# brech1/keaki

Measured on AMD Instinct MI355X. Metric: BN254 G1 scalar-mults/sec on 2^24-point MSM (per GPU), higher is better.
Workload: dtype u32 limbs, 256-bit Montgomery modular integer (9 x 29-bit lazy limbs in the bucket kernel, 8 x 32 elsewhere)

## Files before the change

### bench_tools/dbg/sort_harness.hip

```cpp
#include <hip/hip_runtime.h>
#include <cstdio>
#include <vector>
#ifdef KEAKI_STAMP
__device__ unsigned long long g_stamp[4096];
#define STAMP(cond, i) do { if (cond) g_stamp[(i)] = __builtin_readcyclecounter(); } while (0)
#endif
#include "msm.hip.h"
using namespace bn254;
__global__ void k_fill(u32* p, size_t nwords) {
  size_t i = (size_t)blockIdx.x * blockDim.x + threadIdx.x;
  if (i >= nwords) return;
  unsigned long long z = (i + 1) * 0x9E3779B97F4A7C15ull;
  z = (z ^ (z >> 30)) * 0xBF58476D1CE4E5B9ull; z = (z ^ (z >> 27)) * 0x94D049BB133111EBull; z ^= z >> 31;
  u32 v = (u32)z;
  if ((i & 7) == 7) v &= 0x0FFFFFFFu;
  p[i] = v;
}
#define CK(x) do { hipError_t e_ = (x); if (e_ != hipSuccess) { printf("%s: %s\n", #x, hipGetErrorString(e_)); return 1; } } while (0)
int main(int argc, char** argv) {
  const int log2n = argc > 1 ? atoi(argv[1]) : 24;
  const size_t n = (size_t)1 << log2n;
  MsmPlan plan = msm_make_plan(n, 22);
  MsmShape s = plan.s; s.stride = (u32)n;
  size_t nb = plan.max_b;
  PartShape ps;
  if (!part_make_shape(n, s.W, nb, &ps, argc > 2 ? atoi(argv[2]) : -1, argc > 3 ? atoi(argv[3]) : -1, argc > 4 ? atoi(argv[4]) : -1)) { printf("shape\n"); return 1; }
  printf("n=2^%d W=%u c=%u nbins=%u shift=%u hb=%u nf=%u tile=%u ntiles=%u te=%u geom=%u\n", log2n, s.W, s.c, ps.nbins, ps.shift, ps.hb, ps.nf, ps.tile, ps.ntiles, ps.te, ps.geom);
  const size_t pairs = n * s.W;
  u32 *scal, *tiles, *sorted, *counts, *segoff, *bin_total; u16* tstart; uint2* cellmeta; BinMeta* bins; v4u_t* segtab;
  CK(hipMalloc(&scal, n * 32)); CK(hipMalloc(&tiles, (size_t)ps.ntiles * ps.te * 4)); CK(hipMalloc(&sorted, pairs * 4)); CK(hipMalloc(&counts, nb * 4));
  CK(hipMalloc(&segoff, part_max_chunks(pairs, ps.nbins) * ps.nf * 4)); CK(hipMalloc(&segtab, nb * 16)); CK(hipMalloc(&bin_total, ps.nbins * 4));
  CK(hipMalloc(&tstart, (size_t)ps.ntiles * (ps.nbins + 1) * 2)); CK(hipMalloc(&cellmeta, (size_t)ps.nbins * ps.ntiles * 8)); CK(hipMalloc(&bins, ps.nbins * sizeof(BinMeta)));
  hipLaunchKernelGGL(k_fill, dim3((n * 8 + 255) / 256), dim3(256), 0, 0, scal, n * 8);
  CK(hipDeviceSynchronize());
  hipEvent_t ev[6]; for (auto& e : ev) CK(hipEventCreate(&e));
  int ncu = 256;
  for (int it = 0; it < 4; it++) {
    CK(hipEventRecord(ev[0]));
    hipLaunchKernelGGL(k_tile_sort<12>, dim3(ps.ntiles < (u32)ncu ? ps.ntiles : ncu), dim3(T1_THREADS), 0, 0, (const Fr*)scal, s, ps, tiles, tstart);
    CK(hipEventRecord(ev[1]));
    hipLaunchKernelGGL(k_cell_prefix, dim3(ps.nbins), dim3(1024), 0, 0, (const u16*)tstart, ps, cellmeta, bin_total);
    CK(hipEventRecord(ev[2]));
    hipLaunchKernelGGL(k_bin_scan, dim3(1), dim3(1024), 0, 0, (const u32*)bin_total, ps.nbins, bins);
    CK(hipEventRecord(ev[3]));
#define CS(L, R, Q) hipLaunchKernelGGL((k_chunk_sort<L, R, Q>), dim3(ps.nbins), dim3(C2_THREADS), 0, 0, (const u32*)tiles, (const uint2*)cellmeta, (const BinMeta*)bins, s, ps, (u32)nb, sorted, segtab, segoff, counts)
    switch (ps.geom) { case 0: CS(8, 1, 16); break; case 1: CS(16, 1, 16); break; case 2: CS(16, 2, 8); break; default: CS(16, 4, 4); break; }
    CK(hipEventRecord(ev[4]));
    CK(hipDeviceSynchronize());
    float a, b, c, d;
    CK(hipEventElapsedTime(&a, ev[0], ev[1])); CK(hipEventElapsedTime(&b, ev[1], ev[2])); CK(hipEventElapsedTime(&c, ev[2], ev[3])); CK(hipEventElapsedTime(&d, ev[3], ev[4]));
    printf("tile_sort %.3f  cell_prefix %.3f  bin_scan %.3f  chunk_sort %.3f ms\n", a, b, c, d);
  }
  std::vector<u32> hc(nb); CK(hipMemcpy(hc.data(), counts, nb * 4, hipMemcpyDeviceToHost));
  unsigned long long tot = 0; for (u32 v : hc) tot += v;
  printf("sum of bucket counts %llu (pairs %zu minus zero digits)\n", tot, pairs);
#ifdef KEAKI_STAMP
  std::vector<unsigned long long> st(4096);
  CK(hipMemcpyFromSymbol(st.data(), HIP_SYMBOL(g_stamp), 4096 * 8));
  printf("chunk_sort stamps (one workgroup), cycles between marks per chunk:\n");
  for (int k = 0; k < 8; k++) {
    printf(" chunk %d:", k);
    for (int i = 1; i < 12; i++) { long long d = (long long)(st[k * 16 + i] - st[k * 16 + i - 1]); printf(" %lld", st[k * 16 + i] ? d : -1); }
    printf("  | slow=%llu odd lanes=%llu last odd grp/c0=%llx\n", st[k * 16 + 12], st[k * 16 + 13], st[k * 16 + 14]);
  }
  printf("tile_sort stamps (one workgroup, first tiles):\n");
  for (int k = 0; k < 4; k++) {
    printf(" tile %d:", k);
    for (int i = 1; i < 10; i++) { long long d = (long long)(st[2048 + k * 16 + i] - st[2048 + k * 16 + i - 1]); printf(" %lld", st[2048 + k * 16 + i] ? d : -1); }
// ... 6 lines not shown
```

### keaki_amd/csrc/api.hip

```cpp
#include "internal.h"

#include <algorithm>
#include <set>
#include <utility>
#include <vector>

using namespace keaki_internal;

struct keaki_hip_srs_g1 {
  const void* d = nullptr;
  size_t n = 0;
  bool owned = false;
  int device = -1;
  std::recursive_mutex mu;
  keaki_hip_ctx* acct = nullptr;
  size_t fk_bytes = 0;
  void* table = nullptr;
  size_t table_bytes = 0;
  int c_table = 0;
  void* fk_hat_s = nullptr;
  int fk_log2d = -1;
};
struct keaki_hip_srs_g2 {
  const void* d = nullptr;
// ... 312 lines not shown
#define KEAKI_SRC_HASH "unknown"
#endif
#ifdef KEAKI_DIAG
const char* keaki_hip_version(void) { return "keaki-hip 0.3 (gfx950) DIAGNOSTIC BUILD (diag_row_mask available: not the product) src=" KEAKI_SRC_HASH; }
#else
const char* keaki_hip_version(void) { return "keaki-hip 0.3 (gfx950) src=" KEAKI_SRC_HASH; }
#endif

extern "C++" {
namespace {
void tune_from_env(Tuning& t) {
  auto geti = [](const char* name, long long& out) { const char* e = getenv(name); if (!e || !*e) return false; out = atoll(e); return true; };
  long long v;
  if (geti("KEAKI_MSM_C", v)) t.msm_c = (int)v;
  if (geti("KEAKI_MSM_C_SHARED", v)) t.msm_c_shared = (int)v;
  if (geti("KEAKI_REDUCE_L", v)) t.reduce_l = (int)v;
  if (geti("KEAKI_PART_SHIFT", v)) t.part_shift = (int)v;
  if (geti("KEAKI_ACC_U29", v)) t.acc_u29 = v != 0;
  if (geti("KEAKI_ACC_U29_G2", v)) t.acc_u29_g2 = v != 0;
  if (geti("KEAKI_ACC_NT", v)) t.acc_nt = v != 0;
  if (geti("KEAKI_ACC_PREFETCH", v)) t.acc_prefetch = v != 0;
  if (geti("KEAKI_ACC_IDXQ", v)) t.acc_idxq = v != 0;
  if (geti("KEAKI_CS_MASKED", v)) t.cs_masked = v != 0;
  if (geti("KEAKI_FK_UNIFORM", v)) t.fk_uniform = v != 0;
  if (geti("KEAKI_FK_GTAB", v)) t.fk_gtab = v != 0;
  if (geti("KEAKI_FK_ADDSUB29", v)) t.fk_addsub29 = v != 0;
  if (geti("KEAKI_FK_RADIX4", v)) t.fk_radix4 = v != 0;
  if (geti("KEAKI_FB_OCC1", v)) t.fb_occ1 = v != 0;
  if (geti("KEAKI_MSM_SHORT_TABLES", v)) t.msm_short_tables = (int)v;
  if (geti("KEAKI_PAIR_WIDE_MAX", v)) t.pair_wide_max = (int)v;
  if (geti("KEAKI_PAIR_TWO_WAVES", v)) t.pair_two_waves = v != 0;
  if (geti("KEAKI_GT_WB_B", v)) t.gt_wb_b = (int)v;
  if (geti("KEAKI_ENCAP_GT", v)) t.encap_gt = v;
  if (geti("KEAKI_HOST_PREFAULT", v)) t.host_prefault = v != 0;
  if (geti("KEAKI_PIPE_CHUNKS", v)) t.pipe_chunks = v != 0;
  if (geti("KEAKI_MSM_PIPE_CHUNKS", v)) t.msm_pipe_chunks = (int)v;
  if (geti("KEAKI_MSM_PIPE_MIN", v)) t.msm_pipe_min = v;
  if (geti("KEAKI_MSM_PIPE_GROWTH", v)) t.msm_pipe_growth = (int)v;
}
struct BufClass { DevBuf* b; int cls; };
std::vector<BufClass> all_bufs(keaki_hip_ctx* ctx) {
  std::vector<BufClass> v;
  for (DevBuf* b : {&ctx->digits, &ctx->hist, &ctx->offsets, &ctx->cursor, &ctx->sorted, &ctx->buckets, &ctx->acc29, &ctx->partials, &ctx->wsums, &ctx->bsums,
                    &ctx->tmp_a, &ctx->tmp_b, &ctx->tmp_c, &ctx->io_a, &ctx->io_b, &ctx->io_c, &ctx->io_d, &ctx->io_e, &ctx->perm, &ctx->heavy,
                    &ctx->pair_ws, &ctx->verify_io, &ctx->g2gen_lines, &ctx->fk_tab, &ctx->g2pow_lines, &ctx->g2pow_pts})
    v.push_back({b, 1});
// ... 62 lines not shown
  thread_local std::string copy;
  keaki_hip_ctx* c = const_cast<keaki_hip_ctx*>(ctx);
  std::lock_guard<std::recursive_mutex> lock_(c->mu);
  copy = c->err;
  return copy.c_str();
}

keaki_status keaki_hip_ctx_set_option(keaki_hip_ctx* ctx, const char* name, int64_t value) {
  if (!ctx) return KEAKI_ERR_BAD_ARG;
  std::lock_guard<std::recursive_mutex> lock_(ctx->mu);
  if (!name) return fail(ctx, KEAKI_ERR_BAD_ARG, "ctx_set_option: name is null");
  Tuning& t = ctx->tune;
  const std::string k(name);
  if (k == "msm_c") t.msm_c = (int)value;
  else if (k == "msm_c_shared") t.msm_c_shared = (int)value;
  else if (k == "reduce_l") t.reduce_l = (int)value;
  else if (k == "part_shift") t.part_shift = (int)value;
  else if (k == "acc_u29") t.acc_u29 = value != 0;
  else if (k == "acc_u29_g2") t.acc_u29_g2 = value != 0;
  else if (k == "acc_nt") t.acc_nt = value != 0;
  else if (k == "acc_prefetch") t.acc_prefetch = value != 0;
  else if (k == "acc_idxq") t.acc_idxq = value != 0;
  else if (k == "cs_masked") t.cs_masked = value != 0;
  else if (k == "fk_uniform") t.fk_uniform = value != 0;
  else if (k == "fk_gtab") t.fk_gtab = value != 0;
  else if (k == "fk_addsub29") t.fk_addsub29 = value != 0;
  else if (k == "fk_radix4") t.fk_radix4 = value != 0;
  else if (k == "fb_occ1") t.fb_occ1 = value != 0;
  else if (k == "msm_short_tables") t.msm_short_tables = (int)value;
  else if (k == "pair_wide_max") t.pair_wide_max = (int)value;
  else if (k == "pair_two_waves") t.pair_two_waves = value != 0;
  else if (k == "gt_wb_b") {
    if (value != 0 && (value < 8 || value > 22 || gt_table_powers((uint32_t)value) > 320)) return fail(ctx, KEAKI_ERR_BAD_ARG, "ctx_set_option: gt_wb_b = %lld out of range", (long long)value);
    if ((int)value != t.gt_wb_b) { ctx->gt_b_ready = false; ctx->gt_b_fallback = false; }
    t.gt_wb_b = (int)value;
  } else if (k == "encap_gt") t.encap_gt = value;
  else if (k == "host_prefault") t.host_prefault = value != 0;
  else if (k == "pipe_chunks") t.pipe_chunks = value != 0;
#ifdef KEAKI_DIAG
  else if (k == "diag_row_mask") t.diag_row_mask = (unsigned)value;
#endif
  else if (k == "msm_pipe_chunks") t.msm_pipe_chunks = (int)value;
  else if (k == "msm_pipe_min") t.msm_pipe_min = value;
  else if (k == "msm_pipe_growth") t.msm_pipe_growth = (int)value;
  else return fail(ctx, KEAKI_ERR_BAD_ARG, "ctx_set_option: unknown option '%s'", name);
  return KEAKI_OK;
// ... 1084 lines not shown
```

### keaki_amd/csrc/internal.h

```cpp
#pragma once
#include <hip/hip_runtime.h>

#include <cstdarg>
#include <cstdio>
#include <cstdlib>
#include <atomic>
#include <cstring>
#include <functional>
#include <mutex>
#include <string>
#include <utility>
#include <vector>

#include "../../include/keaki_hip.h"

namespace keaki_internal {

struct DevBuf {
  void* p = nullptr;
  size_t cap = 0;
};

}

namespace keaki_internal {
struct Tuning {
  int msm_c = 0;
  int msm_c_shared = 0;
  int msm_short_tables = -1;
  int reduce_l = 0;
  int part_shift = -1;
  bool acc_u29 = true;
  bool acc_u29_g2 = true;
  bool acc_prefetch = true;
  bool acc_idxq = true;
  bool cs_masked = true;
  bool acc_nt = false;
  bool fk_uniform = true;
  bool fk_gtab = true;
  bool fk_radix4 = true;
  bool fk_addsub29 = true;
  bool fb_occ1 = false;
  int pair_wide_max = -1;
  bool pair_two_waves = true;
  int gt_wb_b = 0;
  long long encap_gt = -1;
  bool host_prefault = true;
  bool pipe_chunks = true;
  int msm_pipe_chunks = -1;
  long long msm_pipe_min = 1 << 20;
  int msm_pipe_growth = 160;
#ifdef KEAKI_DIAG
  unsigned diag_row_mask = 0;
#endif
  size_t alloc_limit = 0;
};
}

struct keaki_hip_ctx {
// ... 155 lines not shown
```

### keaki_amd/csrc/msm.hip.h

```cpp
#pragma once
#include <type_traits>
#include "bn254_curve.hip.h"
#include "fq29.hip.h"
#include "xyzz29.hip.h"
#include "jac29.hip.h"
#include "xyzz29_g2.hip.h"

namespace bn254 {

typedef uint16_t u16;
typedef u32 v4u_t __attribute__((ext_vector_type(4)));
constexpr u32 DIGIT_NONE = 0xFFFFFFFFu;
#ifndef STAMP
#define STAMP(cond, i) do { } while (0)
#endif

struct MsmShape {
  u32 n;
  u32 c;
  u32 W;
  u32 k;
  u32 stride;
};
KDEV u32 msm_width(const MsmShape& s, u32 w) { return w < s.k ? s.c : s.c - 1; }
// ... 63 lines not shown
#pragma unroll
  for (u32 w = 0; w < W; w++) {
    const u32 off = P::offset(w), wd = P::width(w), j = off >> 5, sh = off & 31;
    const u32 lo = v[j], hi = j + 1 < 8 ? v[j + 1] : 0u;
    const u32 d = (sh + wd <= 32 ? lo >> sh : __builtin_amdgcn_alignbit(hi, lo, sh)) & ((1u << wd) - 1u);
    const u32 full = 1u << wd, half = full >> 1;
    const u32 coef = d + carry;
    if (w == W - 1) {
      code[w] = coef ? coef - 1u : DIGIT_NONE;
    } else {
      const bool neg = coef > half;
      carry = neg ? 1u : 0u;
      code[w] = neg ? (coef != full ? ((full - coef - 1u) | 0x80000000u) : DIGIT_NONE) : (coef ? coef - 1u : DIGIT_NONE);
    }
  }
}

template <class Emit>
KDEV void msm_for_each_digit(const Fr& k, const MsmShape& s, Emit emit) {
  u32 v[8];
  fp_from_mont<FrParams>(v, k);
  msm_for_each_digit_canon(v, s, emit);
}

constexpr u32 T1_THREADS = 1024;
constexpr u32 T1_PER = 3;
constexpr u32 T1_CAP = 36864;
constexpr u32 PART_MAX_BINS = 2048;
constexpr u32 C2_THREADS = 1024;
constexpr u32 C2_CAP = 32768;
constexpr u32 PART_MAX_FINE_SHIFT = 11;
constexpr u32 PART_MAX_FINE = 1u << PART_MAX_FINE_SHIFT;
constexpr u32 SEG_INLINE = 4;
constexpr u32 TE_WPOS = 12, TE_SIGN = 19, TE_FINE = 20, TE_VALID = 0x80000000u;

struct PartShape {
  u32 nbins, lb;
  u32 shift, hb;
  u32 nf;
  u32 tile;
  u32 ntiles;
  u32 te;
  u32 geom;
};
KDEV u32 part_bin(const PartShape& ps, u32 g) { return (g >> ps.shift) & (ps.nbins - 1u); }
KDEV u32 part_fine(const PartShape& ps, u32 g) { return ((g >> (ps.shift + ps.lb)) << ps.shift) | (g & ((1u << ps.shift) - 1u)); }
// ... 127 lines not shown
          const u32 g = (s.stride ? 0u : msm_bucket_base(s, w)) + (cd & 0x7FFFFFFFu);
          const u32 pos = atomicAdd(&cur[ok ? part_bin(ps, g) : PART_MAX_BINS + (t & 63u)], 1u);
          ent[ok ? pos : T1_CAP + (t & 63u)] = TE_VALID | (part_fine(ps, g) << TE_FINE) | ((cd >> 31) << TE_SIGN) | (w << TE_WPOS) | li;
        }
      } else if (act[p]) {
        msm_for_each_digit_canon(canon[p], s, [&](u32 w, u32 cd) {
          const u32 g = (s.stride ? 0u : msm_bucket_base(s, w)) + (cd & 0x7FFFFFFFu);
          const u32 pos = atomicAdd(&cur[part_bin(ps, g)], 1u);
          ent[pos] = TE_VALID | (part_fine(ps, g) << TE_FINE) | ((cd >> 31) << TE_SIGN) | (w << TE_WPOS) | li;
        });
      }
    }
    STAMP(blockIdx.x == 100 && t == 0 && sk < 4, 2048 + sk * 16 + 5);
    lds_barrier();
    STAMP(blockIdx.x == 100 && t == 0 && sk < 4, 2048 + sk * 16 + 6);
    u32* dst = tiles + (size_t)tile * ps.te;
#pragma unroll 4
    for (u32 q = t; q < m; q += T1_THREADS) dst[q] = ent[q];
    STAMP(blockIdx.x == 100 && t == 0 && sk < 4, 2048 + sk * 16 + 7);
  }
}

static __global__ void __launch_bounds__(1024) k_cell_prefix(const u16* __restrict__ tstart, PartShape ps, uint2* __restrict__ cellmeta,
                                                             u32* __restrict__ bin_total) {
  __shared__ u32 a[4096];
  __shared__ u32 wsum[16];
  const u32 b = blockIdx.x, t = threadIdx.x;
  u32 carry = 0;
  for (u32 base = 0; base < ps.ntiles; base += 4096) {
    u32 st[4], ln[4];
#pragma unroll
    for (u32 k = 0; k < 4; k++) {
      const u32 tile = base + 4 * t + k;
      st[k] = 0; ln[k] = 0;
      if (tile < ps.ntiles) {
        const u16* row = tstart + (size_t)tile * (ps.nbins + 1) + b;
        st[k] = row[0];
        ln[k] = (u32)row[1] - st[k];
      }
      a[4 * t + k] = ln[k];
    }
    const u32 tot = lds_exclusive_scan4(a, 4096, wsum);
#pragma unroll
    for (u32 k = 0; k < 4; k++) {
      const u32 tile = base + 4 * t + k;
      if (tile < ps.ntiles) cellmeta[(size_t)b * ps.ntiles + tile] = make_uint2(carry + a[4 * t + k], st[k] | (ln[k] << 16));
    }
    carry += tot;
    lds_barrier();
  }
  if (t == 0) bin_total[b] = carry;
}
struct BinMeta {
  u32 img_base, chunk_first, nch, total;
};
static __global__ void __launch_bounds__(1024) k_bin_scan(const u32* __restrict__ bin_total, u32 nbins, BinMeta* __restrict__ bins) {
  __shared__ u32 a[2048];
  __shared__ u32 c[2048];
  __shared__ u32 wsum[16];
  const u32 t = threadIdx.x;
  u32 tt[2];
#pragma unroll
  for (u32 k = 0; k < 2; k++) {
    const u32 b = 2 * t + k;
    tt[k] = b < nbins ? bin_total[b] : 0u;
    a[b] = tt[k];
    c[b] = (tt[k] + C2_CAP - 1) / C2_CAP;
  }
  lds_exclusive_scan4(a, 2048, wsum);
  lds_exclusive_scan4(c, 2048, wsum);
#pragma unroll
  for (u32 k = 0; k < 2; k++) {
    const u32 b = 2 * t + k;
    if (b < nbins) bins[b] = {a[b], c[b], (tt[k] + C2_CAP - 1) / C2_CAP, tt[k]};
  }
}

constexpr u32 C2_META = 2048;
KDEV u32 chunk_payload(u32 en, u32 ibase, u32 stride) {
  return (((en >> TE_SIGN) & 1u) << 31) | (ibase + (en & ((1u << TE_WPOS) - 1u)) + ((en >> TE_WPOS) & ((1u << (TE_SIGN - TE_WPOS)) - 1u)) * stride);
}
template <int PHASE>
KDEV void chunk_slow(const u32* __restrict__ tiles, const uint2* __restrict__ cm, const PartShape& ps, u32 stride, u32 c0, u32 lo, u32 hi, u32* hist,
                     u32* pay, u32* sh_next) {
  const u32 grp = threadIdx.x >> 4, l16 = threadIdx.x & 15;
  for (u32 c = c0 + grp; c < ps.ntiles; c += C2_THREADS / 16) {
    const uint2 m = cm[c];
    const u32 len = m.y >> 16;
    if (PHASE == 0 && m.x + len > hi && l16 == 0) atomicMin(sh_next, c);
    if (m.x > hi || (m.x == hi && len)) break;
    const u32 j0 = m.x < lo ? lo - m.x : 0u, j1 = hi - m.x < len ? hi - m.x : len;
    const u32* src = tiles + (size_t)c * ps.te + (m.y & 0xFFFFu);
    for (u32 j = j0 + l16; j < j1; j += 16) {
      const u32 en = src[j];
      const u32 f = (en >> TE_FINE) & (PART_MAX_FINE - 1u);
      if (PHASE == 0) {
        atomicAdd(&hist[f], 1u);
      } else {
        const u32 pos = atomicAdd(&hist[f], 1u);
        pay[pos] = chunk_payload(en, c * ps.tile, stride);
      }
    }
  }
}
template <u32 L, u32 R, u32 Q, bool MASKED = true>
static __global__ void __launch_bounds__(C2_THREADS) k_chunk_sort(const u32* __restrict__ tiles, const uint2* __restrict__ cellmeta,
                                                                  const BinMeta* __restrict__ bins, MsmShape s, PartShape ps, u32 nbuckets_total,
                                                                  u32* __restrict__ sorted, v4u_t* __restrict__ segtab, u32* __restrict__ segoff,
                                                                  u32* __restrict__ bucket_counts) {
  constexpr u32 GROUPS = C2_THREADS / L, CELLS = GROUPS * Q, CAPC = 4 * L * R, NB = 4, QB = Q / NB;
  static_assert(CELLS <= C2_META && Q * R * 4 <= 64 && Q <= 32 && Q % NB == 0 && PART_MAX_FINE == 2 * C2_THREADS, "gather shape");
  __shared__ u32 pay[C2_CAP + 64];
  __shared__ uint2 meta[C2_META];
  __shared__ u32 hist[PART_MAX_FINE + 64];
  __shared__ u32 wsum[C2_THREADS / 64];
  __shared__ u32 sh_next, sh_odd;
  const u32 b = blockIdx.x, t = threadIdx.x, nf = ps.nf;
  const BinMeta bm = bins[b];
  const uint2* cm = cellmeta + (size_t)b * ps.ntiles;
  u32 tot[2] = {0, 0};
  u32 c0 = 0;
  for (u32 f = t; f < PART_MAX_FINE + 64; f += C2_THREADS) hist[f] = 0;
#pragma unroll
  for (u32 i = 0; i < C2_META / C2_THREADS; i++) {
    const u32 ci = t + i * C2_THREADS;
    if (ci < CELLS) meta[ci] = ci < ps.ntiles ? cm[ci] : make_uint2(0xFFFFFFFFu, 0u);
  }
  if (t == 0) { sh_next = ps.ntiles; sh_odd = 0; }
  lds_barrier();
  for (u32 k = 0; k < bm.nch; k++) {
    const u32 lo = k * C2_CAP, hi = bm.total - lo < C2_CAP ? bm.total : lo + C2_CAP;
    u32 tk = t;
    asm volatile("" : "+v"(tk));
    const u32 grp = tk / L, ll = tk % L, dummy = PART_MAX_FINE + (tk & 63u);
    STAMP(b == 100 && t == 0 && k < 8, k * 16 + 0);
    const size_t span = (size_t)(ps.ntiles - c0) * ps.te * 4;
    const __amdgpu_buffer_rsrc_t img = __builtin_amdgcn_make_buffer_rsrc((void*)(tiles + (size_t)c0 * ps.te), 0,
                                                                       span < 0xFFFFFFF0ull ? (u32)span : 0xFFFFFFF0u, 0x00020000);
    auto fetch = [&](u32 tt, u32 q0, u32 (&e)[QB][R][4], u32& longcells, u32& cand, bool& odd) {
      const u32 grp = tt / L, ll = tt % L;
#pragma unroll
// ... 149 lines not shown
    STAMP(b == 100 && t == 0 && k < 8, k * 16 + 7);
    u32 tw = threadIdx.x;
    asm volatile("" : "+v"(tw));
    u32* dst = sorted + bm.img_base + lo;
#pragma unroll 4
    for (u32 q = tw; q < hi - lo; q += C2_THREADS) dst[q] = pay[q];
    for (u32 f = tw; f < PART_MAX_FINE + 64; f += C2_THREADS) hist[f] = 0;
    if (k + 1 < bm.nch) {
#pragma unroll
      for (u32 i = 0; i < C2_META / C2_THREADS; i++) if (tw + i * C2_THREADS < CELLS) meta[tw + i * C2_THREADS] = mnext[i];
    }
    if (t == 0) { sh_next = ps.ntiles; sh_odd = 0; }
    c0 = c_next;
    STAMP(b == 100 && t == 0 && k < 8, k * 16 + 8);
    lds_barrier();
  }
  u32 te = threadIdx.x;
  asm volatile("" : "+v"(te));
#pragma unroll
  for (u32 i = 0; i < 2; i++) {
    const u32 f = 2 * te + i, g = part_bucket(ps, b, f);
    if (f < nf && g < nbuckets_total) {
      bucket_counts[g] = tot[i];
      for (u32 kk = bm.nch; kk < SEG_INLINE; kk++) reinterpret_cast<u32*>(segtab)[(size_t)g * SEG_INLINE + kk] = 0u;
    }
  }
}

struct SortView {
  const u32* sorted;
  const BinMeta* bins;
  const v4u_t* segtab;
  const u32* segoff;
  PartShape ps;
};
struct SegWalker {
  u32 pos, left;
  u32 w0, w1, w2, w3;
  u32 c, nch;
  u32 img_base, o;
};
KDEV void seg_init(SegWalker& w, const SortView& v, u32 t) {
  const BinMeta bm = v.bins[part_bin(v.ps, t)];
  const v4u_t sw = v.segtab[t];
  w.w0 = sw[0]; w.w1 = sw[1]; w.w2 = sw[2]; w.w3 = sw[3];
  w.img_base = bm.img_base;
  w.o = bm.chunk_first * v.ps.nf + part_fine(v.ps, t);
  w.nch = bm.nch;
// ... 74 lines not shown
  __shared__ u32 wsum[SCAN_THREADS / 64];
  u32 lane = threadIdx.x & 63, wid = threadIdx.x >> 6;
  u32 x = v;
#pragma unroll
  for (int o = 1; o < 64; o <<= 1) {
    u32 y = __shfl_up(x, o, 64);
    if (lane >= (u32)o) x += y;
  }
  if (lane == 63) wsum[wid] = x;
  __syncthreads();
  u32 base = 0, tot = 0;
#pragma unroll
  for (u32 k = 0; k < SCAN_THREADS / 64; k++) {
    u32 s = wsum[k];
    if (k < wid) base += s;
    tot += s;
  }
  __syncthreads();
  *total = tot;
  return base + x - v;
}


constexpr u32 CNT_BINS = 1024;
constexpr u32 HEAVY_MIN = 8192, HEAVY_SLICE = 16384;
struct HeavyList {
  u32 n;
  u32 nslices;
};
static __global__ void __launch_bounds__(256) k_cnt_hist(const u32* __restrict__ counts, u32 nb, u32* __restrict__ ghist, HeavyList* __restrict__ hv,
                                                         u32 hv_cap, u32 hv_slice_cap, u32* __restrict__ hv_bucket, u32* __restrict__ hv_first,
                                                         u32* __restrict__ hv_owner) {
  __shared__ u32 h[CNT_BINS];
  for (u32 b = threadIdx.x; b < CNT_BINS; b += 256) h[b] = 0;
  __syncthreads();
  const u32 base = blockIdx.x * 1024;
  for (u32 t = threadIdx.x; t < 1024; t += 256) {
    u32 g = base + t;
    if (g < nb) {
      u32 c = counts[g];
      atomicAdd(&h[c < CNT_BINS - 1 ? c : CNT_BINS - 1], 1u);
      if (c >= HEAVY_MIN) {
        const u32 nsl = (c + HEAVY_SLICE - 1) / HEAVY_SLICE;
        const u32 slot = atomicAdd(&hv->n, 1u);
        if (slot < hv_cap) {
          const u32 first = atomicAdd(&hv->nslices, nsl);
          hv_bucket[slot] = g;
          hv_first[slot] = first;
          for (u32 k = 0; k < nsl && first + k < hv_slice_cap; k++) hv_owner[first + k] = slot;
        }
      }
    }
  }
  __syncthreads();
  for (u32 b = threadIdx.x; b < CNT_BINS; b += 256) if (h[b]) atomicAdd(&ghist[b], h[b]);
}
static __global__ void __launch_bounds__(CNT_BINS) k_cnt_offsets(const u32* __restrict__ ghist, u32* __restrict__ start) {
  __shared__ u32 sh[CNT_BINS];
  u32 b = threadIdx.x;
  sh[b] = ghist[CNT_BINS - 1 - b];
  __syncthreads();
  for (u32 o = 1; o < CNT_BINS; o <<= 1) {
    u32 v = b >= o ? sh[b - o] : 0u;
    __syncthreads();
    sh[b] += v;
    __syncthreads();
  }
  start[CNT_BINS - 1 - b] = sh[b] - ghist[CNT_BINS - 1 - b];
}
static __global__ void __launch_bounds__(256) k_cnt_scatter(const u32* __restrict__ counts, u32 nb, u32* __restrict__ cursor ,
                                                            u32* __restrict__ perm) {
  __shared__ u32 h[CNT_BINS];
  for (u32 b = threadIdx.x; b < CNT_BINS; b += 256) h[b] = 0;
  __syncthreads();
  const u32 base = blockIdx.x * 1024;
  u32 bin[4], rank[4];
#pragma unroll
  for (u32 k = 0; k < 4; k++) {
    u32 g = base + threadIdx.x + 256 * k;
    bin[k] = CNT_BINS;
    if (g < nb) { u32 c = counts[g]; bin[k] = c < CNT_BINS - 1 ? c : CNT_BINS - 1; rank[k] = atomicAdd(&h[bin[k]], 1u); }
  }
  __syncthreads();
  for (u32 b = threadIdx.x; b < CNT_BINS; b += 256) { u32 c = h[b]; if (c) h[b] = atomicAdd(&cursor[b], c); }
  __syncthreads();
#pragma unroll
  for (u32 k = 0; k < 4; k++) {
    u32 g = base + threadIdx.x + 256 * k;
    if (bin[k] != CNT_BINS) perm[h[bin[k]] + rank[k]] = g;
  }
}


constexpr u32 HEAVY_GRID = 2048, HEAVY_COMBINE_GRID = 512;
template <class F>
__global__ void __launch_bounds__(256) k_msm_heavy(const Aff<F>* __restrict__ points, SortView v, const u32* __restrict__ counts,
                                                   const HeavyList* __restrict__ hv, u32 hv_slice_cap, const u32* __restrict__ hv_bucket,
                                                   const u32* __restrict__ hv_first, const u32* __restrict__ hv_owner, Xyzz<F>* __restrict__ slices) {
  __shared__ Xyzz<F> sh[256];
  __shared__ u32 seg_pos[256], seg_n[256];
  __shared__ u32 nlist;
  const u32 total = min(hv->nslices, hv_slice_cap);
  for (u32 sid = blockIdx.x; sid < total; sid += gridDim.x) {
    const u32 slot = hv_owner[sid];
    const u32 t = hv_bucket[slot];
    const u32 cnt = counts[t];
    const u32 lo = (sid - hv_first[slot]) * HEAVY_SLICE, hi = min(cnt, lo + HEAVY_SLICE);
// ... 462 lines not shown
```

### keaki_amd/csrc/msm_host.hip.h

```cpp
#pragma once
#include <algorithm>
#include <functional>
#include <type_traits>
#include <vector>
#include "internal.h"
#include "msm.hip.h"

namespace keaki_internal {
using namespace bn254;

inline int choose_window(size_t n, int forced = 0) {
  if (forced >= 3 && forced <= 24) return forced;
  if (n < 32) return 3;
  double best = 1e300;
  int bc = 3;
  for (int c = 3; c <= 22; c++) {
    MsmPlan p = msm_make_plan(n, c);
    if (p.nb > ((size_t)PART_MAX_BINS << PART_MAX_FINE_SHIFT)) continue;
    double cost = (double)n * p.s.W + 2.8 * (double)p.nb;
    if ((double)p.nb < 131072.0) cost *= 131072.0 / (double)p.nb;
    if (cost < best) { best = cost; bc = c; }
  }
  return bc;
}
// ... 54 lines not shown
    q.cm_bytes = (size_t)q.ps.nbins * q.ps.ntiles * sizeof(uint2);
    q.bt_bytes = ((size_t)q.ps.nbins * 4 + 15) & ~(size_t)15;
    q.bm_bytes = (size_t)q.ps.nbins * sizeof(BinMeta);
    q.sg_bytes = nb * sizeof(v4u_t);
    q.ts_bytes = (size_t)q.ps.ntiles * (q.ps.nbins + 1) * 2;
    w_digits = std::max(w_digits, (size_t)q.ps.ntiles * q.ps.te * 4);
    w_sorted = std::max(w_sorted, q.pairs * 4 + 64);
    w_offsets = std::max(w_offsets, q.max_chunks * q.ps.nf * 4);
    w_cursor = std::max(w_cursor, q.cm_bytes + q.bt_bytes + q.bm_bytes + q.sg_bytes + q.ts_bytes);
    w_pairs = std::max(w_pairs, q.pairs);
  }
  if (w_total != n) return fail(ctx, KEAKI_ERR_BAD_ARG, "msm: the chunks cover %zu of %zu pairs", w_total, n);
  bool u29 = false;
  if constexpr (std::is_same<F, Fq>::value) u29 = ctx->tune.acc_u29;
  if constexpr (std::is_same<F, Fq2>::value) u29 = ctx->tune.acc_u29_g2;
  bool lazy_state = K > 1 && u29 && std::is_same<F, Fq>::value;
  ST_TRY(reserve(ctx, ctx->digits, w_digits));
  ST_TRY(reserve(ctx, ctx->sorted, w_sorted));
  ST_TRY(reserve(ctx, ctx->hist, nb * 4));
  ST_TRY(reserve(ctx, ctx->offsets, w_offsets));
  ST_TRY(reserve(ctx, ctx->cursor, w_cursor));
  ST_TRY(reserve(ctx, ctx->buckets, nb * sizeof(Xyzz<F>)));
  ST_TRY(reserve(ctx, ctx->partials, ((size_t)rs.W * chunks + (size_t)rs.W * 256) * sizeof(Xyzz<F>)));
  ST_TRY(reserve(ctx, ctx->perm, nb * 4 + 2 * CNT_BINS * 4 + sizeof(HeavyList)));
  const u32 hv_cap = (u32)(w_pairs / HEAVY_MIN + 1), hv_slice_cap = (u32)(hv_cap + w_pairs / HEAVY_SLICE + 1);
  const size_t hv_hdr = ((2 * (size_t)hv_cap + hv_slice_cap) * 4 + 255) & ~(size_t)255;
  ST_TRY(reserve(ctx, ctx->heavy, hv_hdr + (size_t)hv_slice_cap * sizeof(Xyzz<F>)));
  if (lazy_state) {
    const keaki_status st29 = reserve(ctx, ctx->acc29, nb * sizeof(Acc29));
    if (st29 == KEAKI_ERR_OOM) { lazy_state = false; u29 = false; ctx->err.clear(); }
    else if (st29 != KEAKI_OK) return st29;
  }
  u32 *tiles = (u32*)ctx->digits.p, *sorted = (u32*)ctx->sorted.p, *hist = (u32*)ctx->hist.p;
  u32* segoff = (u32*)ctx->offsets.p;
  Xyzz<F>* buckets = (Xyzz<F>*)ctx->buckets.p;
  Xyzz<F>* partials = (Xyzz<F>*)ctx->partials.p;
  Acc29* state29 = lazy_state ? (Acc29*)ctx->acc29.p : nullptr;
  u32* perm = (u32*)ctx->perm.p;
  u32 *gstart = perm + nb, *ghist = gstart + CNT_BINS;
  HeavyList* hv = (HeavyList*)(ghist + CNT_BINS);
  u32 *hv_bucket = (u32*)ctx->heavy.p, *hv_first = hv_bucket + hv_cap, *hv_owner = hv_first + hv_cap;
  Xyzz<F>* hv_slices = (Xyzz<F>*)((char*)ctx->heavy.p + hv_hdr);
  for (size_t j = 0; j < K; j++) {
    const Pass& q = passes[j];
    const PartShape& ps = q.ps;
    if (pipe && pipe->stage) ST_TRY(pipe->stage(j));
    MsmShape sj = s;
    sj.n = (u32)q.m;
    const Fr* scal = (const Fr*)d_scalars + q.lo;
    const Aff<F>* pts = d_points + q.lo;
    const bool first = j == 0, last = j + 1 == K;
    uint2* cellmeta = (uint2*)ctx->cursor.p;
    u32* bin_total = (u32*)((char*)ctx->cursor.p + q.cm_bytes);
    BinMeta* bins = (BinMeta*)((char*)bin_total + q.bt_bytes);
    v4u_t* segtab = (v4u_t*)((char*)bins + q.bm_bytes);
    u16* tstart = (u16*)((char*)segtab + q.sg_bytes);
    {
      const dim3 g1(ps.ntiles < ctx->n_cu ? ps.ntiles : ctx->n_cu), b1(T1_THREADS);
#define KEAKI_TILE_SORT(WS) hipLaunchKernelGGL(k_tile_sort<WS>, g1, b1, 0, st, scal, sj, ps, tiles, tstart)
      switch (s.W) {
        case 11: KEAKI_TILE_SORT(11); break;
        case 12: KEAKI_TILE_SORT(12); break;
        case 13: KEAKI_TILE_SORT(13); break;
        case 14: KEAKI_TILE_SORT(14); break;
        case 15: KEAKI_TILE_SORT(15); break;
        case 16: KEAKI_TILE_SORT(16); break;
        default: KEAKI_TILE_SORT(0); break;
      }
#undef KEAKI_TILE_SORT
    }
    ST_TRY(launch_check(ctx, "tile_sort"));
    hipLaunchKernelGGL(k_cell_prefix, dim3(ps.nbins), dim3(1024), 0, st, (const u16*)tstart, ps, cellmeta, bin_total);
    hipLaunchKernelGGL(k_bin_scan, dim3(1), dim3(1024), 0, st, (const u32*)bin_total, ps.nbins, bins);
    {
#define KEAKI_CHUNK_SORT1(L, R, Q, M)                                                                                                                  \
  hipLaunchKernelGGL((k_chunk_sort<L, R, Q, M>), dim3(ps.nbins), dim3(C2_THREADS), 0, st, (const u32*)tiles, (const uint2*)cellmeta, (const BinMeta*)bins, sj, \
                     ps, (u32)nb, sorted, segtab, segoff, hist)
#define KEAKI_CHUNK_SORT(L, R, Q) do { if (ctx->tune.cs_masked) KEAKI_CHUNK_SORT1(L, R, Q, true); else KEAKI_CHUNK_SORT1(L, R, Q, false); } while (0)
      switch (ps.geom) {
        case 0: KEAKI_CHUNK_SORT(8, 1, 16); break;
        case 1: KEAKI_CHUNK_SORT(16, 1, 16); break;
        case 2: KEAKI_CHUNK_SORT(16, 2, 8); break;
        default: KEAKI_CHUNK_SORT(16, 4, 4); break;
      }
#undef KEAKI_CHUNK_SORT1
#undef KEAKI_CHUNK_SORT
    }
    ST_TRY(launch_check(ctx, "chunk_sort"));
#ifdef KEAKI_DIAG
    if (ctx->tune.diag_row_mask) hipLaunchKernelGGL(k_diag_mask_rows, dim3(4096), dim3(256), 0, st, sorted, (size_t)q.pairs, (u32)ctx->tune.diag_row_mask);
#endif
    const SortView view = {sorted, bins, segtab, segoff, ps};
    HIP_TRY(ctx, hipMemsetAsync(ghist, 0, CNT_BINS * 4 + sizeof(HeavyList), st));
    hipLaunchKernelGGL(k_cnt_hist, dim3(cdiv(nb, 1024)), dim3(256), 0, st, (const u32*)hist, (u32)nb, ghist, hv, hv_cap, hv_slice_cap, hv_bucket, hv_first,
                       hv_owner);
    hipLaunchKernelGGL(k_cnt_offsets, dim3(1), dim3(CNT_BINS), 0, st, (const u32*)ghist, gstart);
    hipLaunchKernelGGL(k_cnt_scatter, dim3(cdiv(nb, 1024)), dim3(256), 0, st, (const u32*)hist, (u32)nb, gstart, perm);
    ST_TRY(launch_check(ctx, "cnt_sort"));
    if (ctx->timing && last) (void)hipEventRecord(ctx->ev[1], st);
    const dim3 ga(cdiv(nb, 256)), ba(256);
    bool done = false;
    if constexpr (std::is_same<F, Fq>::value) {
      if (u29) {
#define KEAKI_ACC(NT, MODE) hipLaunchKernelGGL((k_msm_accumulate_g1_u29<NT, MODE>), ga, ba, 0, st, pts, view, (const u32*)hist, (const u32*)perm, (u32)nb, buckets, state29)
        if (K == 1) {
          if (ctx->tune.acc_nt) KEAKI_ACC(1, ACC_WHOLE);
          else if (!ctx->tune.acc_prefetch)
            hipLaunchKernelGGL((k_msm_accumulate_g1_u29<0, ACC_WHOLE, 0>), ga, ba, 0, st, pts, view, (const u32*)hist, (const u32*)perm, (u32)nb, buckets, state29);
          else if (!ctx->tune.acc_idxq)
            hipLaunchKernelGGL((k_msm_accumulate_g1_u29<0, ACC_WHOLE, 1>), ga, ba, 0, st, pts, view, (const u32*)hist, (const u32*)perm, (u32)nb, buckets, state29);
          else KEAKI_ACC(0, ACC_WHOLE);
        }
        else if (first) KEAKI_ACC(0, ACC_FIRST);
        else if (!last) KEAKI_ACC(0, ACC_MIDDLE);
        else KEAKI_ACC(0, ACC_LAST);
#undef KEAKI_ACC
        done = true;
      }
    }
    if constexpr (std::is_same<F, Fq2>::value) {
// ... 68 lines not shown
```

Before: 1.012 billion.

## Fold bin scan and count histogram into chunk sort to drop launches

Adds a sort_fold option, on by default, that removes the separate k_bin_scan, memset, k_cnt_hist and k_cnt_offsets launches. Each chunk_sort block computes its own prefix of bin totals by summing the totals of all earlier bins, and accumulates the bucket-count histogram into a global array. Zeroing moves into cell_prefix, while the histogram scan and heavy-bucket detection move into cnt_scatter. This trades several small serial launches for redundant per-block prefix work (a quadratic-ish read of bin totals) plus global atomics.

```diff
diff --git a/bench_tools/dbg/sort_harness.hip b/bench_tools/dbg/sort_harness.hip
--- a/bench_tools/dbg/sort_harness.hip
+++ b/bench_tools/dbg/sort_harness.hip
@@ -39,11 +39,11 @@
     CK(hipEventRecord(ev[0]));
     hipLaunchKernelGGL(k_tile_sort<12>, dim3(ps.ntiles < (u32)ncu ? ps.ntiles : ncu), dim3(T1_THREADS), 0, 0, (const Fr*)scal, s, ps, tiles, tstart);
     CK(hipEventRecord(ev[1]));
-    hipLaunchKernelGGL(k_cell_prefix, dim3(ps.nbins), dim3(1024), 0, 0, (const u16*)tstart, ps, cellmeta, bin_total);
+    hipLaunchKernelGGL(k_cell_prefix, dim3(ps.nbins), dim3(1024), 0, 0, (const u16*)tstart, ps, cellmeta, bin_total, bins, nullptr, 0u);
     CK(hipEventRecord(ev[2]));
     hipLaunchKernelGGL(k_bin_scan, dim3(1), dim3(1024), 0, 0, (const u32*)bin_total, ps.nbins, bins);
     CK(hipEventRecord(ev[3]));
-#define CS(L, R, Q) hipLaunchKernelGGL((k_chunk_sort<L, R, Q>), dim3(ps.nbins), dim3(C2_THREADS), 0, 0, (const u32*)tiles, (const uint2*)cellmeta, (const BinMeta*)bins, s, ps, (u32)nb, sorted, segtab, segoff, counts)
+#define CS(L, R, Q) hipLaunchKernelGGL((k_chunk_sort<L, R, Q>), dim3(ps.nbins), dim3(C2_THREADS), 0, 0, (const u32*)tiles, (const uint2*)cellmeta, bins, s, ps, (u32)nb, sorted, segtab, segoff, counts, nullptr)
     switch (ps.geom) { case 0: CS(8, 1, 16); break; case 1: CS(16, 1, 16); break; case 2: CS(16, 2, 8); break; default: CS(16, 4, 4); break; }
     CK(hipEventRecord(ev[4]));
     CK(hipDeviceSynchronize());
diff --git a/keaki_amd/csrc/api.hip b/keaki_amd/csrc/api.hip
--- a/keaki_amd/csrc/api.hip
+++ b/keaki_amd/csrc/api.hip
@@ -358,6 +358,7 @@
   if (geti("KEAKI_ACC_PREFETCH", v)) t.acc_prefetch = v != 0;
   if (geti("KEAKI_ACC_IDXQ", v)) t.acc_idxq = v != 0;
   if (geti("KEAKI_CS_MASKED", v)) t.cs_masked = v != 0;
+  if (geti("KEAKI_SORT_FOLD", v)) t.sort_fold = v != 0;
   if (geti("KEAKI_FK_UNIFORM", v)) t.fk_uniform = v != 0;
   if (geti("KEAKI_FK_GTAB", v)) t.fk_gtab = v != 0;
   if (geti("KEAKI_FK_ADDSUB29", v)) t.fk_addsub29 = v != 0;
@@ -466,6 +467,7 @@
   else if (k == "acc_prefetch") t.acc_prefetch = value != 0;
   else if (k == "acc_idxq") t.acc_idxq = value != 0;
   else if (k == "cs_masked") t.cs_masked = value != 0;
+  else if (k == "sort_fold") t.sort_fold = value != 0;
   else if (k == "fk_uniform") t.fk_uniform = value != 0;
   else if (k == "fk_gtab") t.fk_gtab = value != 0;
   else if (k == "fk_addsub29") t.fk_addsub29 = value != 0;
diff --git a/keaki_amd/csrc/internal.h b/keaki_amd/csrc/internal.h
--- a/keaki_amd/csrc/internal.h
+++ b/keaki_amd/csrc/internal.h
@@ -35,6 +35,7 @@
   bool acc_prefetch = true;
   bool acc_idxq = true;
   bool cs_masked = true;
+  bool sort_fold = true;
   bool acc_nt = false;
   bool fk_uniform = true;
   bool fk_gtab = true;
diff --git a/keaki_amd/csrc/msm.hip.h b/keaki_amd/csrc/msm.hip.h
--- a/keaki_amd/csrc/msm.hip.h
+++ b/keaki_amd/csrc/msm.hip.h
@@ -109,6 +109,10 @@
   fp_from_mont<FrParams>(v, k);
   msm_for_each_digit_canon(v, s, emit);
 }
+
+struct BinMeta {
+  u32 img_base, chunk_first, nch, total;
+};
 
 constexpr u32 T1_THREADS = 1024;
 constexpr u32 T1_PER = 3;
@@ -282,10 +286,13 @@
 }
 
 static __global__ void __launch_bounds__(1024) k_cell_prefix(const u16* __restrict__ tstart, PartShape ps, uint2* __restrict__ cellmeta,
-                                                             u32* __restrict__ bin_total) {
+                                                             u32* __restrict__ bin_total, BinMeta* __restrict__ bins, u32* __restrict__ zero,
+                                                             u32 nzero) {
   __shared__ u32 a[4096];
   __shared__ u32 wsum[16];
   const u32 b = blockIdx.x, t = threadIdx.x;
+  if (zero && b == 0)
+    for (u32 i = t; i < nzero; i += 1024) zero[i] = 0;
   u32 carry = 0;
   for (u32 base = 0; base < ps.ntiles; base += 4096) {
     u32 st[4], ln[4];
@@ -309,11 +316,11 @@
     carry += tot;
     lds_barrier();
   }
-  if (t == 0) bin_total[b] = carry;
-}
-struct BinMeta {
-  u32 img_base, chunk_first, nch, total;
-};
+  if (t == 0) {
+    if (zero) bins[b].total = carry;
+    else bin_total[b] = carry;
+  }
+}
 static __global__ void __launch_bounds__(1024) k_bin_scan(const u32* __restrict__ bin_total, u32 nbins, BinMeta* __restrict__ bins) {
   __shared__ u32 a[2048];
   __shared__ u32 c[2048];
@@ -333,6 +340,24 @@
   for (u32 k = 0; k < 2; k++) {
     const u32 b = 2 * t + k;
     if (b < nbins) bins[b] = {a[b], c[b], (tt[k] + C2_CAP - 1) / C2_CAP, tt[k]};
+  }
+}
+
+constexpr u32 CNT_BINS = 1024;
+constexpr u32 HEAVY_MIN = 8192, HEAVY_SLICE = 16384;
+struct HeavyList {
+  u32 n;
+  u32 nslices;
+};
+constexpr u32 CNT_GHIST = CNT_BINS, CNT_HV = 2 * CNT_BINS, CNT_WORDS = CNT_HV + sizeof(HeavyList) / 4;
+KDEV void cnt_note_heavy(u32 g, u32 c, HeavyList* hv, u32 hv_cap, u32 hv_slice_cap, u32* hv_bucket, u32* hv_first, u32* hv_owner) {
+  const u32 nsl = (c + HEAVY_SLICE - 1) / HEAVY_SLICE;
+  const u32 slot = atomicAdd(&hv->n, 1u);
+  if (slot < hv_cap) {
+    const u32 first = atomicAdd(&hv->nslices, nsl);
+    hv_bucket[slot] = g;
+    hv_first[slot] = first;
+    for (u32 k = 0; k < nsl && first + k < hv_slice_cap; k++) hv_owner[first + k] = slot;
   }
 }
 
@@ -363,11 +388,11 @@
     }
   }
 }
-template <u32 L, u32 R, u32 Q, bool MASKED = true>
+template <u32 L, u32 R, u32 Q, bool MASKED = true, bool FOLD = false>
 static __global__ void __launch_bounds__(C2_THREADS) k_chunk_sort(const u32* __restrict__ tiles, const uint2* __restrict__ cellmeta,
-                                                                  const BinMeta* __restrict__ bins, MsmShape s, PartShape ps, u32 nbuckets_total,
+                                                                  BinMeta* __restrict__ bins, MsmShape s, PartShape ps, u32 nbuckets_total,
                                                                   u32* __restrict__ sorted, v4u_t* __restrict__ segtab, u32* __restrict__ segoff,
-                                                                  u32* __restrict__ bucket_counts) {
+                                                                  u32* __restrict__ bucket_counts, u32* __restrict__ cnt) {
   constexpr u32 GROUPS = C2_THREADS / L, CELLS = GROUPS * Q, CAPC = 4 * L * R, NB = 4, QB = Q / NB;
   static_assert(CELLS <= C2_META && Q * R * 4 <= 64 && Q <= 32 && Q % NB == 0 && PART_MAX_FINE == 2 * C2_THREADS, "gather shape");
   __shared__ u32 pay[C2_CAP + 64];
@@ -375,8 +400,28 @@
   __shared__ u32 hist[PART_MAX_FINE + 64];
   __shared__ u32 wsum[C2_THREADS / 64];
   __shared__ u32 sh_next, sh_odd;
+  __shared__ u32* sh_cnt;
   const u32 b = blockIdx.x, t = threadIdx.x, nf = ps.nf;
-  const BinMeta bm = bins[b];
+  BinMeta bm;
+  if constexpr (FOLD) {
+    u32 img = 0, chf = 0;
+    for (u32 i = t; i < b; i += C2_THREADS) { const u32 x = bins[i].total; img += x; chf += (x + C2_CAP - 1) / C2_CAP; }
+#pragma unroll
+    for (int o = 32; o >= 1; o >>= 1) { img += __shfl_xor(img, o, 64); chf += __shfl_xor(chf, o, 64); }
+    if ((t & 63u) == 0) { wsum[t >> 6] = img; hist[t >> 6] = chf; }
+    const u32 total = __builtin_amdgcn_readfirstlane(bins[b].total);
+    if (t == 0) sh_cnt = cnt;
+    lds_barrier();
+    img = 0; chf = 0;
+#pragma unroll
+    for (u32 w = 0; w < C2_THREADS / 64; w++) { img += wsum[w]; chf += hist[w]; }
+    img = __builtin_amdgcn_readfirstlane(img); chf = __builtin_amdgcn_readfirstlane(chf);
+    bm = {img, chf, (total + C2_CAP - 1) / C2_CAP, total};
+    if (t == 0) { bins[b].img_base = img; bins[b].chunk_first = chf; bins[b].nch = bm.nch; }
+    lds_barrier();
+  } else {
+    bm = bins[b];
+  }
   const uint2* cm = cellmeta + (size_t)b * ps.ntiles;
   u32 tot[2] = {0, 0};
   u32 c0 = 0;
@@ -572,8 +617,14 @@
     const u32 f = 2 * te + i, g = part_bucket(ps, b, f);
     if (f < nf && g < nbuckets_total) {
       bucket_counts[g] = tot[i];
+      if constexpr (FOLD) atomicAdd(&hist[tot[i] < CNT_BINS - 1 ? tot[i] : CNT_BINS - 1], 1u);
       for (u32 kk = bm.nch; kk < SEG_INLINE; kk++) reinterpret_cast<u32*>(segtab)[(size_t)g * SEG_INLINE + kk] = 0u;
     }
+  }
+  if constexpr (FOLD) {
+    u32* const ghist = sh_cnt + CNT_GHIST;
+    lds_barrier();
+    for (u32 x = te; x < CNT_BINS; x += C2_THREADS) if (hist[x]) atomicAdd(&ghist[x], hist[x]);
   }
 }
 
@@ -694,12 +745,6 @@
 }
 
 
-constexpr u32 CNT_BINS = 1024;
-constexpr u32 HEAVY_MIN = 8192, HEAVY_SLICE = 16384;
-struct HeavyList {
-  u32 n;
-  u32 nslices;
-};
 static __global__ void __launch_bounds__(256) k_cnt_hist(const u32* __restrict__ counts, u32 nb, u32* __restrict__ ghist, HeavyList* __restrict__ hv,
                                                          u32 hv_cap, u32 hv_slice_cap, u32* __restrict__ hv_bucket, u32* __restrict__ hv_first,
                                                          u32* __restrict__ hv_owner) {
@@ -712,16 +757,7 @@
     if (g < nb) {
       u32 c = counts[g];
       atomicAdd(&h[c < CNT_BINS - 1 ? c : CNT_BINS - 1], 1u);
-      if (c >= HEAVY_MIN) {
-        const u32 nsl = (c + HEAVY_SLICE - 1) / HEAVY_SLICE;
-        const u32 slot = atomicAdd(&hv->n, 1u);
-        if (slot < hv_cap) {
-          const u32 first = atomicAdd(&hv->nslices, nsl);
-          hv_bucket[slot] = g;
-          hv_first[slot] = first;
-          for (u32 k = 0; k < nsl && first + k < hv_slice_cap; k++) hv_owner[first + k] = slot;
-        }
-      }
+      if (c >= HEAVY_MIN) cnt_note_heavy(g, c, hv, hv_cap, hv_slice_cap, hv_bucket, hv_first, hv_owner);
     }
   }
   __syncthreads();
@@ -741,8 +777,16 @@
   start[CNT_BINS - 1 - b] = sh[b] - ghist[CNT_BINS - 1 - b];
 }
 static __global__ void __launch_bounds__(256) k_cnt_scatter(const u32* __restrict__ counts, u32 nb, u32* __restrict__ cursor ,
-                                                            u32* __restrict__ perm) {
+                                                            u32* __restrict__ perm, HeavyList* __restrict__ hv, u32 hv_cap, u32 hv_slice_cap,
+                                                            u32* __restrict__ hv_bucket, u32* __restrict__ hv_first, u32* __restrict__ hv_owner,
+                                                            const u32* __restrict__ ghist) {
   __shared__ u32 h[CNT_BINS];
+  __shared__ u32 st[CNT_BINS];
+  __shared__ u32 wsum[4];
+  if (hv) {
+    for (u32 b = threadIdx.x; b < CNT_BINS; b += 256) st[b] = ghist[CNT_BINS - 1 - b];
+    lds_exclusive_scan4(st, CNT_BINS, wsum);
+  }
   for (u32 b = threadIdx.x; b < CNT_BINS; b += 256) h[b] = 0;
   __syncthreads();
   const u32 base = blockIdx.x * 1024;
@@ -751,10 +795,13 @@
   for (u32 k = 0; k < 4; k++) {
     u32 g = base + threadIdx.x + 256 * k;
     bin[k] = CNT_BINS;
-    if (g < nb) { u32 c = counts[g]; bin[k] = c < CNT_BINS - 1 ? c : CNT_BINS - 1; rank[k] = atomicAdd(&h[bin[k]], 1u); }
+    if (g < nb) {
+      u32 c = counts[g]; bin[k] = c < CNT_BINS - 1 ? c : CNT_BINS - 1; rank[k] = atomicAdd(&h[bin[k]], 1u);
+      if (hv && c >= HEAVY_MIN) cnt_note_heavy(g, c, hv, hv_cap, hv_slice_cap, hv_bucket, hv_first, hv_owner);
+    }
   }
   __syncthreads();
-  for (u32 b = threadIdx.x; b < CNT_BINS; b += 256) { u32 c = h[b]; if (c) h[b] = atomicAdd(&cursor[b], c); }
+  for (u32 b = threadIdx.x; b < CNT_BINS; b += 256) { u32 c = h[b]; if (c) h[b] = atomicAdd(&cursor[b], c) + (hv ? st[CNT_BINS - 1 - b] : 0u); }
   __syncthreads();
 #pragma unroll
   for (u32 k = 0; k < 4; k++) {
diff --git a/keaki_amd/csrc/msm_host.hip.h b/keaki_amd/csrc/msm_host.hip.h
--- a/keaki_amd/csrc/msm_host.hip.h
+++ b/keaki_amd/csrc/msm_host.hip.h
@@ -100,7 +100,7 @@
   ST_TRY(reserve(ctx, ctx->cursor, w_cursor));
   ST_TRY(reserve(ctx, ctx->buckets, nb * sizeof(Xyzz<F>)));
   ST_TRY(reserve(ctx, ctx->partials, ((size_t)rs.W * chunks + (size_t)rs.W * 256) * sizeof(Xyzz<F>)));
-  ST_TRY(reserve(ctx, ctx->perm, nb * 4 + 2 * CNT_BINS * 4 + sizeof(HeavyList)));
+  ST_TRY(reserve(ctx, ctx->perm, nb * 4 + CNT_WORDS * 4));
   const u32 hv_cap = (u32)(w_pairs / HEAVY_MIN + 1), hv_slice_cap = (u32)(hv_cap + w_pairs / HEAVY_SLICE + 1);
   const size_t hv_hdr = ((2 * (size_t)hv_cap + hv_slice_cap) * 4 + 255) & ~(size_t)255;
   ST_TRY(reserve(ctx, ctx->heavy, hv_hdr + (size_t)hv_slice_cap * sizeof(Xyzz<F>)));
@@ -117,6 +117,7 @@
   u32* perm = (u32*)ctx->perm.p;
   u32 *gstart = perm + nb, *ghist = gstart + CNT_BINS;
   HeavyList* hv = (HeavyList*)(ghist + CNT_BINS);
+  const bool fold = ctx->tune.sort_fold;
   u32 *hv_bucket = (u32*)ctx->heavy.p, *hv_first = hv_bucket + hv_cap, *hv_owner = hv_first + hv_cap;
   Xyzz<F>* hv_slices = (Xyzz<F>*)((char*)ctx->heavy.p + hv_hdr);
   for (size_t j = 0; j < K; j++) {
@@ -148,13 +149,15 @@
 #undef KEAKI_TILE_SORT
     }
     ST_TRY(launch_check(ctx, "tile_sort"));
-    hipLaunchKernelGGL(k_cell_prefix, dim3(ps.nbins), dim3(1024), 0, st, (const u16*)tstart, ps, cellmeta, bin_total);
-    hipLaunchKernelGGL(k_bin_scan, dim3(1), dim3(1024), 0, st, (const u32*)bin_total, ps.nbins, bins);
+    hipLaunchKernelGGL(k_cell_prefix, dim3(ps.nbins), dim3(1024), 0, st, (const u16*)tstart, ps, cellmeta, bin_total, bins, fold ? gstart : nullptr,
+                       CNT_WORDS);
+    if (!fold) hipLaunchKernelGGL(k_bin_scan, dim3(1), dim3(1024), 0, st, (const u32*)bin_total, ps.nbins, bins);
     {
-#define KEAKI_CHUNK_SORT1(L, R, Q, M)                                                                                                                  \
-  hipLaunchKernelGGL((k_chunk_sort<L, R, Q, M>), dim3(ps.nbins), dim3(C2_THREADS), 0, st, (const u32*)tiles, (const uint2*)cellmeta, (const BinMeta*)bins, sj, \
-                     ps, (u32)nb, sorted, segtab, segoff, hist)
-#define KEAKI_CHUNK_SORT(L, R, Q) do { if (ctx->tune.cs_masked) KEAKI_CHUNK_SORT1(L, R, Q, true); else KEAKI_CHUNK_SORT1(L, R, Q, false); } while (0)
+#define KEAKI_CHUNK_SORT1(L, R, Q, M, FD)                                                                                                              \
+  hipLaunchKernelGGL((k_chunk_sort<L, R, Q, M, FD>), dim3(ps.nbins), dim3(C2_THREADS), 0, st, (const u32*)tiles, (const uint2*)cellmeta, bins, sj, ps, \
+                     (u32)nb, sorted, segtab, segoff, hist, fold ? gstart : nullptr)
+#define KEAKI_CHUNK_SORT2(L, R, Q, M) do { if (fold) KEAKI_CHUNK_SORT1(L, R, Q, M, true); else KEAKI_CHUNK_SORT1(L, R, Q, M, false); } while (0)
+#define KEAKI_CHUNK_SORT(L, R, Q) do { if (ctx->tune.cs_masked) KEAKI_CHUNK_SORT2(L, R, Q, true); else KEAKI_CHUNK_SORT2(L, R, Q, false); } while (0)
       switch (ps.geom) {
         case 0: KEAKI_CHUNK_SORT(8, 1, 16); break;
         case 1: KEAKI_CHUNK_SORT(16, 1, 16); break;
@@ -162,6 +165,7 @@
         default: KEAKI_CHUNK_SORT(16, 4, 4); break;
       }
 #undef KEAKI_CHUNK_SORT1
+#undef KEAKI_CHUNK_SORT2
 #undef KEAKI_CHUNK_SORT
     }
     ST_TRY(launch_check(ctx, "chunk_sort"));
@@ -169,11 +173,14 @@
     if (ctx->tune.diag_row_mask) hipLaunchKernelGGL(k_diag_mask_rows, dim3(4096), dim3(256), 0, st, sorted, (size_t)q.pairs, (u32)ctx->tune.diag_row_mask);
 #endif
     const SortView view = {sorted, bins, segtab, segoff, ps};
-    HIP_TRY(ctx, hipMemsetAsync(ghist, 0, CNT_BINS * 4 + sizeof(HeavyList), st));
-    hipLaunchKernelGGL(k_cnt_hist, dim3(cdiv(nb, 1024)), dim3(256), 0, st, (const u32*)hist, (u32)nb, ghist, hv, hv_cap, hv_slice_cap, hv_bucket, hv_first,
-                       hv_owner);
-    hipLaunchKernelGGL(k_cnt_offsets, dim3(1), dim3(CNT_BINS), 0, st, (const u32*)ghist, gstart);
-    hipLaunchKernelGGL(k_cnt_scatter, dim3(cdiv(nb, 1024)), dim3(256), 0, st, (const u32*)hist, (u32)nb, gstart, perm);
+    if (!fold) {
+      HIP_TRY(ctx, hipMemsetAsync(ghist, 0, CNT_BINS * 4 + sizeof(HeavyList), st));
+      hipLaunchKernelGGL(k_cnt_hist, dim3(cdiv(nb, 1024)), dim3(256), 0, st, (const u32*)hist, (u32)nb, ghist, hv, hv_cap, hv_slice_cap, hv_bucket, hv_first,
+                         hv_owner);
+      hipLaunchKernelGGL(k_cnt_offsets, dim3(1), dim3(CNT_BINS), 0, st, (const u32*)ghist, gstart);
+    }
+    hipLaunchKernelGGL(k_cnt_scatter, dim3(cdiv(nb, 1024)), dim3(256), 0, st, (const u32*)hist, (u32)nb, gstart, perm, fold ? hv : nullptr, hv_cap,
+                       hv_slice_cap, hv_bucket, hv_first, hv_owner, (const u32*)ghist);
     ST_TRY(launch_check(ctx, "cnt_sort"));
     if (ctx->timing && last) (void)hipEventRecord(ctx->ev[1], st);
     const dim3 ga(cdiv(nb, 256)), ba(256);
```

Result: no change. 1.011 billion, median of 6 (-0.1%).
